# abdur75648/AI-Camera

Hardware: AMD Instinct MI355X
Metric: end-to-end frames/sec @1280x720, 30 persons/frame (higher is better)
Workload: dtype f16

## Files before the change

ai-camera_amd/csrc/conv_plan.cpp:

```cpp
#include "conv_plan.hpp"

#include <algorithm>
#include <cstdlib>

namespace aic {

static int g_conv_cus = 256;
int conv_cu_budget() { return g_conv_cus; }
void set_conv_cu_budget(int cus) { g_conv_cus = std::max(1, cus); }

static long cdiv(long a, long b) { return (a + b - 1) / b; }
static const long B31 = 1l << 31;

static int tile_run(long ntiles, int max_run) {
    int run = 1;
    long best = -1;
    for (int r = 1; r <= max_run; ++r) {
        const long blocks = (ntiles + r - 1) / r, rounds = (blocks + 255) / 256;
        if (r > 1 && rounds < 4) break;
        const long cost = rounds * r;
        if (best < 0 || cost <= best) best = cost, run = r;
    }
    return run;
}
// ... 274 lines not shown

bool conv_x2_supported(int dtype, const ConvArgs& a, int cin2) {
    const int bke = dtype == AIC_F16 ? 32 : 16;
    const int shape = pp_patch_shape(dtype, a);
    if (shape < 2 || a.Cout % 128 || a.w_tail || a.out_f32 || cin2 <= 0 || cin2 % bke) return false;
    return cin2 / bke < a.Cin / bke;
}

int plan_c64_block(const ConvArgs& c1, const ConvArgs& c2, int cu_budget) {
    static const bool on = [] { const char* e = getenv("AICAM_C64_BLOCK"); return !e || atoi(e) != 0; }();
    auto conv64 = [](const ConvArgs& a) {
        return a.KH == 3 && a.KW == 3 && a.stride == 1 && a.pad == 1 && a.Cin == 64 && a.Cout == 64 && !a.out_f32 && a.Kp == 576 && a.act == 2 &&
               a.Ho == a.H && a.Wo == a.W && (a.x_cs | a.x_coff | a.y_cs | a.y_coff) % 8 == 0;
    };
    if (!on || !conv64(c1) || !conv64(c2) || c1.res_mode != 0 || c2.res_mode != 1) return 0;
    if (c1.W != 32 || c1.H % 4 || c1.H != c2.H || c2.W != 32 || c1.M != c2.M || c1.M < 1500000) return 0;
    if (c2.x != c1.y || c2.x_cs != c1.y_cs || c2.x_coff != c1.y_coff) return 0;
    if (c2.res != c1.x || c2.r_cs != c1.x_cs || c2.r_coff != c1.x_coff) return 0;
    if ((long)c1.M * c1.x_cs >= B31 || (long)c2.M * c2.y_cs >= B31) return 0;
    const int n_img = c1.M / (c1.H * c1.W), cus = (cu_budget + 7) / 8 * 8;
    long best = -1;
    int ipb = 0;
    for (int i = 12; i <= 16; ++i) {
        const long blocks = (n_img + i - 1) / i, rounds = (blocks + cus - 1) / cus;
        const long waste = (rounds * cus - blocks) * 1000 / (rounds * cus);
        if (best < 0 || waste < best) best = waste, ipb = i;
    }
    return ipb;
}

bool plan_c2f16(const ConvArgs& c1, const ConvArgs& m1, const ConvArgs& m2, const ConvArgs& c2) {
    static const bool off = getenv("AICAM_NO_C2F") != nullptr;
    if (off) return false;
    auto one = [](const ConvArgs& c, int cin, int cout, int kp) {
        return c.KH == 1 && c.KW == 1 && c.stride == 1 && c.pad == 0 && c.Cin == cin && c.Cout == cout && c.Kp == kp && c.act == 1 &&
               c.res_mode == 0 && !c.out_f32;
    };
    auto three = [](const ConvArgs& c) {
        return c.KH == 3 && c.KW == 3 && c.stride == 1 && c.pad == 1 && c.Cin == 16 && c.Cout == 16 && c.Kp == 160 && c.act == 1 && !c.out_f32;
    };
    if (!one(c1, 32, 32, 32) || !one(c2, 48, 32, 64) || !three(m1) || !three(m2) || m1.res_mode != 0 || m2.res_mode != 2) return false;
    const int H = c1.H, W = c1.W;
    for (const ConvArgs* c : {&c1, &m1, &m2, &c2})
        if (c->H != H || c->W != W || c->Ho != H || c->Wo != W || c->M != c1.M) return false;
    if (H % 8 || W % 32) return false;
    const void* cat = c1.y;
    if (c1.y_coff != 0 || m1.x != cat || m1.x_coff != 16 || m1.x_cs != c1.y_cs || m2.x != m1.y || m2.x_coff != m1.y_coff || m2.x_cs != m1.y_cs ||
        m2.y != cat || m2.y_coff != 32 || m2.res != cat || m2.r_coff != 16 || m2.r_cs != c1.y_cs || c2.x != cat || c2.x_coff != 0 ||
        c2.x_cs != c1.y_cs || c1.y_cs < 48)
        return false;
    return (c1.x_cs | c1.x_coff | c2.y_cs | c2.y_coff) % 8 == 0;
}

}
```

ai-camera_amd/csrc/conv_plan.hpp:

```cpp
#pragma once
#include "assoc_host.hpp"

namespace aic {

struct ConvArgs {
    const void* x;
    const void* w;
    const float* bias;
    void* y;
    const void* res;
    int x_cs, x_coff, H, W, Cin;
    int y_cs, y_coff, Ho, Wo, Cout;
    int r_cs, r_coff, res_mode, act;
    int KH, KW, stride, pad;
    int Kp;
    int M;
    int out_f32;
    int cout_pad;
    unsigned tap_rows;
    const void* zero;
    int xcd_map;
    const float* bias_init;
    const int* n_dev;
    int k_order;
// ... 3 lines not shown
    int xs_cs, xs_coff, Hs, Ws, Cs;
    const void* w_tail;
    const float* b_tail;
    void* y_tail;
    int t_cout, t_kp, t_y_cs, t_y_coff, t_out_f32, t_act;
    float* t_max; int* t_arg;
    int t_hw, t_a0, t_na;
    float* t_box; int t_w, t_stride;
};

int conv_cu_budget();
void set_conv_cu_budget(int cus);

enum class ConvForm {
    Dma,
    Wide,
    Pp,
    PpPatch,
    SpPatch,
    S2Patch,
    Patch,
    PmPatch,
    C16,
    C32s2Tail,
    Stream1x1,
    C64Resident,
};

struct ConvPlan {
    ConvForm form = ConvForm::Dma;
    int mt = 0, nt = 0, wm = 0, wn = 0;
    int nstage = 0;
    int th = 0, tw = 0;
    int cpp = 0, pitch = 0;
    int kord = 0;
    int g = 0;
    bool tail = false;
    bool x2 = false;
    int run = 1;
    long blocks = 0;
};

int conv_k_order(int dtype, const ConvArgs& a);
ConvPlan plan_conv(int dtype, const ConvArgs& a, int cu_budget);

ConvPlan plan_conv_launch(int dtype, ConvArgs& a, int cu_budget);

bool conv_tail_supported(int dtype, const ConvArgs& lead, const ConvArgs& tail);
bool conv_xs_supported(int dtype, const ConvArgs& a, int cs);
bool conv_x2_supported(int dtype, const ConvArgs& a, int cin2);

int plan_c64_block(const ConvArgs& c1, const ConvArgs& c2, int cu_budget);
bool plan_c2f16(const ConvArgs& cv1, const ConvArgs& m_cv1, const ConvArgs& m_cv2, const ConvArgs& cv2);

}
```

ai-camera_amd/csrc/engine.cpp:

```cpp
#include "engine.hpp"

#include <algorithm>
#include <cmath>
#include <cstdlib>
#include <fstream>

namespace aic {

namespace {

struct Reader {
    const char* p;
    size_t n, off = 0;
    template <class T> const T* take(size_t count) {
        AIC_REQUIRE(off + count * sizeof(T) <= n, AIC_ERR_FORMAT, "engine file truncated");
        const T* r = reinterpret_cast<const T*>(p + off);
        off += count * sizeof(T);
        return r;
    }
};

inline int round_up(int v, int m) { return (v + m - 1) / m * m; }

inline uint16_t f32_to_f16_bits(float f) {
// ... 488 lines not shown
    auto conv_args = [&](size_t k) {
        const int* u = ops[k].v;
        const BufDesc& xb = bufs[u[1]];
        const BufDesc& yb = bufs[u[4]];
        const ConvWeights& w = weights[u[15]];
        ConvArgs a{};
        a.x = xb.p, a.w = w.w.p, a.bias = w.bias.p, a.y = yb.p;
        a.x_cs = xb.c, a.x_coff = u[2], a.H = xb.h, a.W = xb.w, a.Cin = w.cin_eff;
        a.y_cs = yb.c, a.y_coff = u[5], a.Ho = yb.h, a.Wo = yb.w, a.Cout = w.cout;
        a.res = nullptr, a.r_cs = 0, a.r_coff = 0, a.res_mode = u[14], a.act = u[11];
        if (u[14]) { a.res = bufs[u[12]].p, a.r_cs = bufs[u[12]].c, a.r_coff = u[13]; }
        a.KH = w.kh, a.KW = w.kw, a.stride = u[9], a.pad = u[10];
        if (ops[k].xs_buf >= 0) {
            const BufDesc& bs = bufs[ops[k].xs_buf];
            a.xs = bs.p, a.xs_cs = bs.c, a.xs_coff = ops[k].xs_coff, a.Hs = bs.h, a.Ws = bs.w, a.Cs = ops[k].xs_c;
        }
        if (u[16]) {
            const BufDesc& b2 = bufs[u[16] - 1];
            a.x2 = b2.p, a.x2_cs = b2.c, a.x2_coff = u[17], a.H2 = b2.h, a.W2 = b2.w, a.s2 = u[19], a.Cin2 = u[18];
            fl += 2.0 * n * yb.h * yb.w * (double)w.cout * u[18];
            by += ((double)n * yb.h * yb.w * u[18] + (double)w.cout * u[18]) * (dtype == AIC_F16 ? 2 : 4);
        }
        a.Kp = w.Kp, a.M = n * yb.h * yb.w, a.out_f32 = yb.f32, a.cout_pad = w.cout_pad, a.zero = d_zero.p;
        a.tap_rows = 0;
        a.n_dev = n_items_dev;
        for (int kh = 0; kh < w.kh; ++kh) a.tap_rows |= 1u << (kh * w.kw);
        AIC_REQUIRE(w.kh * w.kw <= 25, AIC_ERR_FORMAT, "kernel window larger than 5x5");
        fl += 2.0 * a.M * (double)w.cout * w.cin * w.kh * w.kw;
        by += ((double)n * xb.h * xb.w * w.cin + (double)a.M * w.cout) * (dtype == AIC_F16 ? 2 : 4) +
              (double)w.cout * w.cin * w.kh * w.kw * (dtype == AIC_F16 ? 2 : 4);
        return a;
    };
    auto done = [&](int kind, int n_ops) { st.kind = kind, st.n_ops = n_ops, st.fl = fl, st.by = by; return st; };
    const ConvArgs a = st.a[0] = conv_args(oi);
    bool pair = false;
    ConvArgs a2{};
    if (dtype == AIC_F16 && oi + 1 < op1 && ops[oi + 1].v[0] == OP_CONV && ops[oi + 1].fuse == 0 && a.Cin == 64 && a.Cout == 64 &&
        a.res_mode == 0 && ops[oi + 1].v[14] == 1) {
        const double fl0 = fl, by0 = by;
        a2 = conv_args(oi + 1);
        pair = a2.res == a.x && a2.x == a.y;
        if (!pair) fl = fl0, by = by0;
    }
    if (!pair && dtype == AIC_F16 && oi + 3 < op1 && a.KH == 1 && a.Cin == 32 && a.Cout == 32 && ops[oi + 1].v[0] == OP_CONV &&
        ops[oi + 2].v[0] == OP_CONV && ops[oi + 3].v[0] == OP_CONV && !ops[oi + 1].fuse && !ops[oi + 2].fuse && !ops[oi + 3].fuse) {
        const double fl0 = fl, by0 = by;
        const ConvArgs b1 = conv_args(oi + 1), b2 = conv_args(oi + 2), b3 = conv_args(oi + 3);
        if (plan_c2f16(a, b1, b2, b3)) {
            st.a[1] = b1, st.a[2] = b2, st.a[3] = b3;
            return done(ConvStep::C2f16, 4);
        }
        fl = fl0, by = by0;
    }
    if (const int ipb = pair ? plan_c64_block(a, a2, conv_cu_budget()) : 0) {
        st.a[1] = a2, st.ipb = ipb;
        return done(ConvStep::C64Block, 2);
    }
    if (pair) { fl = 0, by = 0; (void)conv_args(oi); }
    if (o.fuse == 3 && oi + 1 < op1) {
        const double fl0 = fl, by0 = by;
        const ConvArgs t = conv_args(oi + 1);
        if (conv_tail_supported(dtype, a, t)) {
            ConvArgs at = a;
            at.w_tail = t.w, at.b_tail = t.bias, at.y_tail = t.y, at.t_cout = t.Cout, at.t_kp = t.Kp;
            at.t_y_cs = t.y_cs, at.t_y_coff = t.y_coff, at.t_out_f32 = t.out_f32, at.t_act = t.act;
            static const bool cls_reduce_on = getenv("AICAM_NO_CLS_REDUCE") == nullptr;
            static const bool box_decode_on = getenv("AICAM_NO_BOX_DECODE") == nullptr;
            if (reduce_cls && kind == KIND_YOLO && t.out_f32 && t.act == 0 && t.y_coff == 0 && t.y_cs == t.Cout) {
                const bool is_cls = cls_reduce_on && t.Cout == meta[0], is_box = box_decode_on && meta[1] == 16 && t.Cout == 64 && a.Cout == 64 && !is_cls;
                int a0 = 0;
                for (size_t l = 0; l < outs.size() && (is_cls || is_box); ++l) {
                    const int* ov = outs[l].v;
                    const BufDesc& ob = bufs[ov[is_cls ? 1 : 0]];
                    if (ob.p == t.y && ov[3] * ov[4] == t.Ho * t.Wo) {
                        at.t_hw = ov[3] * ov[4], at.t_a0 = a0, at.t_na = n_anchors;
                        if (is_cls) {
                            at.t_max = d_maxlogit.p, at.t_arg = d_labels.p;
                            st.cls_bits |= 1u << l;
                        } else {
                            at.t_box = d_boxes.p, at.t_w = ov[4], at.t_stride = ov[2];
                            st.box_bits |= 1u << l;
                        }
                    }
                    a0 += ov[3] * ov[4];
                }
            }
            st.a[0] = at;
            return done(ConvStep::Tail, 2);
        }
        fl = fl0, by = by0;
    }
    return done(ConvStep::Single, 1);
}

void Model::run_range(size_t op0, size_t op1, int n, hipStream_t s) {
    const bool prof_conv = (dev->prof_mask >> PROF_CONV) & 1u;
    bool span_open = false;
    auto span_close = [&] { if (span_open) { dev->prof_end(PROF_CONV, s); span_open = false; } };
    for (size_t oi = op0; oi < op1; ++oi) {
        const OpDesc& o = ops[oi];
        const int* v = o.v;
        const BufDesc& sb = bufs[v[1]];
        const BufDesc& db = bufs[v[4]];
        if (o.fuse == 2) continue;
        if (o.fuse == 1 || v[0] != OP_CONV) span_close();
        if (o.fuse == 1) {
            const ConvWeights& w = weights[v[15]];
            const int* pv = ops[oi + 1].v;
            const BufDesc& pb = bufs[pv[4]];
            const double fl = 2.0 * n * sb.h * sb.w * 64.0 * 27.0;
            Prof pr(*dev, PROF_CONV_DIRECT, s, fl, (double)n * (sb.h * sb.w * 16.0 + pb.h * pb.w * 128.0));
            launch_reid_stem_pool(sb.p, w.w.p, w.bias.p, pb.p, n, sb.h, sb.w, w.Kp, pb.c, pv[5], in_pix4 ? 4 : 8, s,
                                  (crop_src.frames && in_pix4) ? &crop_src : nullptr, n_items_dev);
            continue;
        }
        if (v[0] == OP_CONV) {
            if (prof_conv && !span_open) { dev->prof_begin(PROF_CONV, s, 0, 0); span_open = true; }
            const ConvStep st = conv_step(oi, op1, n);
            if (prof_conv) dev->prof_account(PROF_CONV, st.fl, st.by);
            switch (st.kind) {
                case ConvStep::C2f16: launch_c2f16(st.a[0], st.a[1], st.a[2], st.a[3], s); break;
                case ConvStep::C64Block: launch_c64_block(st.a[0], st.a[1], st.ipb, s); break;
                case ConvStep::Tail: cls_reduced |= st.cls_bits, box_decoded |= st.box_bits; [[fallthrough]];
                default: launch_conv_igemm(dtype, st.a[0], s);
            }
            oi += st.n_ops - 1;
        } else {
            EltArgs a{};
            a.src = sb.p, a.dst = db.p, a.n = n, a.h = sb.h, a.w = sb.w, a.c = v[3];
            if (emb_host_out && oi + 1 == ops.size() && v[0] == OP_L2NORM && v[4] == outs[0].v[0]) a.dst = emb_host_out;
            a.s_cs = sb.c, a.s_coff = v[2], a.d_cs = db.c, a.d_coff = v[5];
            a.n_dev = n_items_dev;
            Prof pr(*dev, PROF_MISC, s, 0, 0);
            switch (v[0]) {
                case OP_SPPF_POOL: launch_sppf_pool(dtype, a, s); break;
                case OP_UPSAMPLE2X: launch_upsample2x(dtype, a, s); break;
                case OP_MAXPOOL3S2: launch_maxpool3s2(dtype, a, s); break;
                case OP_AVGPOOL: launch_avgpool(dtype, a, s); break;
                case OP_L2NORM: launch_l2norm(dtype, a, s); break;
                default: throw Error(AIC_ERR_FORMAT, "unknown op in engine file");
            }
        }
    }
    span_close();
}

DetArgs Model::det_args(int batch, float conf, float iou, int max_det, const LetterboxGeom* g) {
    AIC_REQUIRE(kind == KIND_YOLO, AIC_ERR_INVALID, "not a YOLO engine");
    AIC_REQUIRE(max_det > 0 && max_det <= max_det_cap, AIC_ERR_CAPACITY, "max_det out of range (1..1024)");
    AIC_REQUIRE(conf > 0.f && conf < 1.f, AIC_ERR_INVALID, "conf_thresh must be in (0,1)");
    DetArgs a{};
    int a0 = 0;
    for (size_t l = 0; l < outs.size(); ++l) {
        const int* v = outs[l].v;
        a.lvl[l].box = reinterpret_cast<const float*>(bufs[v[0]].p);
        a.lvl[l].cls = reinterpret_cast<const float*>(bufs[v[1]].p);
        a.lvl[l].stride = v[2], a.lvl[l].h = v[3], a.lvl[l].w = v[4], a.lvl[l].a0 = a0;
        a.lvl[l].cls_reduced = (cls_reduced >> l) & 1u, a.lvl[l].box_decoded = (box_decoded >> l) & 1u;
        a0 += v[3] * v[4];
    }
    a.n_levels = (int)outs.size(), a.n_anchors = n_anchors, a.nc = meta[0], a.reg_max = meta[1], a.batch = batch;
    a.fast_exp = dtype == AIC_F16;
    a.logit_thr = (float)std::log((double)conf / (1.0 - (double)conf));
    a.iou_thr = iou, a.max_det = max_det;
    a.pad_w = g ? g->pad_w : 0.f, a.pad_h = g ? g->pad_h : 0.f, a.ratio = g ? g->ratio : 1.f;
    a.orig_w = g ? g->src_w : in_w, a.orig_h = g ? g->src_h : in_h;
    a.boxes = d_boxes.p, a.max_logit = d_maxlogit.p, a.labels = d_labels.p, a.keys = nullptr;
    a.n_cand = d_ncand.p, a.num_dets = d_numdets.p;
    a.out_boxes = d_out_boxes.p, a.out_boxes_orig = g ? d_out_boxes_orig.p : nullptr;
    a.out_scores = d_out_scores.p, a.out_labels = d_out_labels.p;
    return a;
}

void Model::decode_nms(int batch, float conf, float iou, int max_det, const LetterboxGeom* g, hipStream_t s, char* host_out) {
// ... 412 lines not shown
```

ai-camera_amd/csrc/engine.hpp:

```cpp
#pragma once
#include "kernels.hpp"

#include <algorithm>
#include <memory>
#include <vector>

namespace aic {

enum { OP_CONV = 1, OP_SPPF_POOL = 2, OP_UPSAMPLE2X = 3, OP_MAXPOOL3S2 = 4, OP_AVGPOOL = 5, OP_L2NORM = 6 };
enum { KIND_YOLO = 1, KIND_REID = 2 };

struct BufDesc { int h, w, c, f32; void* p; size_t per_item; int esize; };
struct ConvWeights { DevBuf<char> w; DevBuf<float> bias; int cout, cin, cin_eff, kh, kw, K, Kp, cout_pad; int cin2 = 0; };
struct OpDesc { int v[20]; int fuse = 0; int xs_buf = -1, xs_coff = 0, xs_c = 0; };
struct OutDesc { int v[8]; };

struct Model {
    Device* dev = nullptr;
    int kind = 0, in_h = 0, in_w = 0, dtype = AIC_F16, max_items = 0;
    int meta[8] = {0};
    std::vector<BufDesc> bufs;
    std::vector<DevBuf<char>> storage;
    std::vector<OpDesc> ops;
    std::vector<ConvWeights> weights;
    std::vector<OutDesc> outs;
    double flops_per_item = 0;
    int n_convs = 0, n_anchors = 0, out_dim = 0;

    int max_det_cap = 0;
    DevBuf<float> d_boxes, d_maxlogit, d_out_boxes, d_out_boxes_orig, d_out_scores;
    DevBuf<int> d_labels, d_ncand, d_numdets, d_out_labels;
    DevBuf<float> d_in_f32;
    DevBuf<uint8_t> d_frames;
    DevBuf<float> d_crop_boxes;
    DevBuf<int> d_valid;
    DevBuf<char> d_zero;

    std::shared_ptr<const std::vector<char>> blob_copy;
    Model(Device& d, const void* blob, size_t nbytes, int dtype_, int max_items_);
    void* input() { return bufs[0].p; }
    bool in_pix4 = false;
    CropSrc crop_src{nullptr, 0, 0, nullptr, nullptr, nullptr};
    const int* n_items_dev = nullptr;
    bool reduce_cls = false;
    unsigned cls_reduced = 0, box_decoded = 0;
    bool input_pix4_ok() const;
    int fast_items() const {
        size_t per = 1;
        for (const OpDesc& o : ops) {
            if (o.v[0] != OP_CONV || o.fuse != 0) continue;
            for (int bi : {o.v[1], o.v[4]}) per = std::max(per, bufs[bi].per_item / (size_t)std::max(bufs[bi].esize, 1));
        }
        const size_t n = std::min<size_t>((size_t)max_items, ((1ull << 31) - 1) / per);
        return (int)(n > 64 && n < (size_t)max_items ? n / 64 * 64 : n);
    }
    void run(int n_items, hipStream_t s);
    void run_frames(const uint8_t* frames, int n, const LetterboxGeom& g, hipStream_t s);
    void run_range(size_t op0, size_t op1, int n, hipStream_t s);
    struct ConvStep {
        enum { Single = 0, Tail = 1, C64Block = 2, C2f16 = 3 };
        int kind = Single, n_ops = 1;
        int ipb = 0;
        unsigned cls_bits = 0, box_bits = 0;
        ConvArgs a[4];
        double fl = 0, by = 0;
    };
    ConvStep conv_step(size_t oi, size_t op1, int n) const;
    struct SideHead { size_t a, b, cut; };
    std::vector<SideHead> side_heads;
    hipStream_t side_stream[2] = {nullptr, nullptr};
    hipEvent_t side_fork[2] = {nullptr, nullptr}, side_join[2] = {nullptr, nullptr};
    bool side_ok = false;
    int side_max_items = 2;
    void plan_side_heads();
    void run_ops(size_t op0, int n, hipStream_t s);
    ~Model();
    DetArgs det_args(int batch, float conf, float iou, int max_det, const LetterboxGeom* g);
    void decode_nms(int batch, float conf, float iou, int max_det, const LetterboxGeom* g, hipStream_t s, char* host_out = nullptr);
    PinBuf<char> h_det;
    float* emb_host_out = nullptr;
    PinBuf<char> h_emb;
    const float* embeddings() const { return reinterpret_cast<const float*>(bufs[outs[0].v[0]].p); }
};

}

struct aic_model { aic::Model m; aic_model(aic::Device& d, const void* b, size_t n, int dt, int mi) : m(d, b, n, dt, mi) {} };
```

ai-camera_amd/csrc/kernels.hpp:

```cpp
#pragma once
#include "common.hpp"
#include "conv_plan.hpp"

namespace aic {

typedef _Float16 half_t;

void launch_conv_igemm(int dtype, const ConvArgs& a, hipStream_t s);
void launch_c64_block(const ConvArgs& c1, const ConvArgs& c2, int ipb, hipStream_t s);
void launch_c2f16(const ConvArgs& cv1, const ConvArgs& m_cv1, const ConvArgs& m_cv2, const ConvArgs& cv2, hipStream_t s);

struct LetterboxGeom;
bool launch_yolo_stem_fused(const uint8_t* frames, int n, const LetterboxGeom& g, const void* w, const float* bias, int Kp, void* y,
                            int y_cs, int y_coff, int Ho, int Wo, hipStream_t s);

struct CropSrc { const uint8_t* frames; int fh, fw; const float* boxes; const int* frame_of; int* valid; };
void launch_reid_stem_pool(const void* x, const void* w, const float* bias, void* y, int n, int H, int W, int Kp, int y_cs,
                           int y_coff, int in_stride, hipStream_t s, const CropSrc* crop = nullptr, const int* n_dev = nullptr);
bool reid_stem2_usable(int H, int W);

struct EltArgs {
    const void* src; void* dst;
    int n, h, w, c;
    int s_cs, s_coff, d_cs, d_coff;
    const int* n_dev;
};
void launch_sppf_pool(int dtype, const EltArgs& a, hipStream_t s);
void launch_upsample2x(int dtype, const EltArgs& a, hipStream_t s);
void launch_maxpool3s2(int dtype, const EltArgs& a, hipStream_t s);
void launch_avgpool(int dtype, const EltArgs& a, hipStream_t s);
void launch_l2norm(int dtype, const EltArgs& a, hipStream_t s);
void launch_nchw_to_nhwc8(int dtype, const float* src, void* dst, int n, int h, int w, hipStream_t s);
void launch_copy_f32(const float* src, float* dst, size_t count, hipStream_t s);

struct LetterboxGeom {
    int src_h, src_w, out_h, out_w, unpad_h, unpad_w, top, left;
    float ratio, pad_w, pad_h;
};
LetterboxGeom letterbox_geometry(int h, int w, int out_h, int out_w);
void launch_letterbox(const uint8_t* frames, int n, const LetterboxGeom& g, int mode, int dtype, void* out,
                      hipStream_t s);
void launch_letterbox_u8(const uint8_t* frame, const LetterboxGeom& g, const int color_bgr[3], uint8_t* out, hipStream_t s);
void launch_crop_resize(const uint8_t* frames, int h, int w, const float* boxes, const int* frame_of, int n,
                        const int* n_dev, int out_h, int out_w, int mode, int dtype, void* out, int* valid,
                        hipStream_t s, bool slack = false);

struct HeadLevel { const float* box; const float* cls; int h, w, stride, a0; int cls_reduced, box_decoded; };
struct DetArgs {
    HeadLevel lvl[4];
    int n_levels, n_anchors, nc, reg_max, batch;
    int fast_exp;
    float logit_thr, iou_thr;
    int max_det;
    float pad_w, pad_h, ratio; int orig_w, orig_h;
    float* boxes;
    float* max_logit;
    int* labels;
    unsigned long long* keys;
    int* n_cand;
    int* num_dets;
    float* out_boxes;
    float* out_boxes_orig;
    float* out_scores;
// ... 61 lines not shown
```

ai-camera_amd/csrc/kernels_conv_c2f.hip:

```cpp
#include "conv_common.hpp"

namespace aic {

namespace {

constexpr int TH = 8, TW = 32;
constexpr int XR = TH + 4, XC = TW + 4;
constexpr int TR = TH + 2, TC = TW + 2;
constexpr int PX = XR * XC * 16, PT = (TR * TC * 16 + 255) / 256 * 256, PY = TH * TW * 16;
static_assert(PX % 256 == 0 && PY % 256 == 0, "plane pitch");
__device__ __forceinline__ int x_slot(int p, int g) {
    return (p & ~7) | ((p & 7) ^ (2 * g));
}
static_assert((XR * XC) % 8 == 0, "swizzle group");
constexpr int LDS_X = 0, LDS_T = 0, LDS_Y1 = LDS_T + 2 * PT, LDS_Y0A = 4 * PX, LDS_Y0B = LDS_Y0A + 2 * PY;
constexpr int LDS_BYTES = LDS_Y0B + 2 * PX;
static_assert(LDS_Y1 + 2 * PY <= 4 * PX, "T and Y1 live in X's place");

}

struct C2fArgs {
    const half_t* x; half_t* y;
    const half_t *w1, *w2, *w3, *w4;
    const float *b1, *b2, *b3, *b4;
// ... 110 lines not shown
            const int oyl = 2 * wv + (tile >> 1), oxl = (tile & 1) * 16 + r;
            const int base = LDS_T + (oyl * TC + oxl) * 16;
            floatx4 acc = bi3;
#pragma unroll
            for (int m = 0; m < 5; ++m)
                acc = __builtin_amdgcn_mfma_f32_16x16x32_f16(w3[m], *reinterpret_cast<const half8*>(smem + base + d[m]), acc, 0, 0, 0);
            const half4 res = *reinterpret_cast<const half4*>(smem + LDS_Y0B + (q >> 1) * PX + ((oyl + 2) * XC + oxl + 2) * 16 + (q & 1) * 8);
            half4 o;
#pragma unroll
            for (int e = 0; e < 4; ++e) o[e] = (half_t)(act_fast<1>(acc[e]) + (float)res[e]);
            *reinterpret_cast<half4*>(smem + LDS_Y1 + (q >> 1) * PY + (oyl * TW + oxl) * 16 + (q & 1) * 8) = o;
        }
    }
    __syncthreads();

    half_t* yg = a.y + (size_t)img * a.H * a.W * a.y_cs + a.y_coff;
#pragma unroll
    for (int tile = 0; tile < 4; ++tile) {
        const int oyl = 2 * wv + (tile >> 1), oxl = (tile & 1) * 16 + r;
        const int a0 = q < 2 ? LDS_Y0A + q * PY + (oyl * TW + oxl) * 16 : LDS_Y0B + (q - 2) * PX + ((oyl + 2) * XC + oxl + 2) * 16;
        const half8 x0 = *reinterpret_cast<const half8*>(smem + a0);
        const half8 x1 = *reinterpret_cast<const half8*>(smem + LDS_Y1 + (q & 1) * PY + (oyl * TW + oxl) * 16);
        float v[2][4];
#pragma unroll
        for (int ct = 0; ct < 2; ++ct) {
            floatx4 acc = {0.f, 0.f, 0.f, 0.f};
            acc = __builtin_amdgcn_mfma_f32_16x16x32_f16(w4[ct][0], x0, acc, 0, 0, 0);
            acc = __builtin_amdgcn_mfma_f32_16x16x32_f16(w4[ct][1], x1, acc, 0, 0, 0);
#pragma unroll
            for (int e = 0; e < 4; ++e) v[ct][e] = act_fast<1>(acc[e] + bi4[ct][e]);
        }
        const half8 o = {(half_t)v[0][0], (half_t)v[0][1], (half_t)v[0][2], (half_t)v[0][3],
                         (half_t)v[1][0], (half_t)v[1][1], (half_t)v[1][2], (half_t)v[1][3]};
        *reinterpret_cast<half8*>(yg + ((size_t)(oy0 + oyl) * a.W + ox0 + oxl) * a.y_cs + 8 * q) = o;
    }
}

void launch_c2f16(const ConvArgs& c1, const ConvArgs& m1, const ConvArgs& m2, const ConvArgs& c2, hipStream_t s) {
    static_assert(TH == 8 && TW == 32, "plan_c2f16 checks the map against 8 x 32 tiles");
    const int H = c1.H, W = c1.W;
    C2fArgs a{};
    a.x = reinterpret_cast<const half_t*>(c1.x), a.y = reinterpret_cast<half_t*>(c2.y);
    a.w1 = reinterpret_cast<const half_t*>(c1.w), a.w2 = reinterpret_cast<const half_t*>(m1.w);
    a.w3 = reinterpret_cast<const half_t*>(m2.w), a.w4 = reinterpret_cast<const half_t*>(c2.w);
    a.b1 = c1.bias, a.b2 = m1.bias, a.b3 = m2.bias, a.b4 = c2.bias;
    a.x_cs = c1.x_cs, a.x_coff = c1.x_coff, a.y_cs = c2.y_cs, a.y_coff = c2.y_coff, a.H = H, a.W = W;
    a.n_img = c1.M / (H * W), a.xcd_map = 1;
    set_lds_limit(c2f16_fused_kernel, LDS_BYTES);
    const int tiles_x = W / TW, tiles_y = H / TH;
    hipLaunchKernelGGL(c2f16_fused_kernel, dim3(a.n_img * tiles_x * tiles_y), dim3(256), (size_t)LDS_BYTES, s, a, tiles_x, tiles_y);
    KCHECK();
}

}
```

ai-camera_amd/hip_engine.py:

```python
from __future__ import annotations

import ctypes as C
import os
import time
from pathlib import Path
from typing import Dict, List, NamedTuple, Tuple

import numpy as np

from . import _lib as L
from . import config

TensorInfo = NamedTuple('TensorInfo', [('name', str), ('dtype', object), ('shape', Tuple[int, ...]), ('is_dynamic', bool)])


def _torch():
    import torch
    return torch


class HipEngine:
    default_conf, default_iou, default_max_det = config.YOLO_CONF_THRESHOLD, config.YOLO_NMS_THRESHOLD, config.YOLO_MAX_DET

    def __init__(self, engine_path, device=None, dtype="fp16", max_items=None, warm_up=True):
# ... 54 lines not shown
        try:
            self.close()
        except Exception:
            pass

    def yolo_infer_np(self, images_nchw, conf=None, iou=None, max_det=None):
        x = L.as_f32(images_nchw)
        b = x.shape[0]
        md = int(max_det or self.max_det)
        nd = np.zeros(b, np.int32)
        boxes, scores, labels = np.zeros((b, md, 4), np.float32), np.zeros((b, md), np.float32), np.zeros((b, md), np.int32)
        L.call("aic_yolo_infer", self._h, L.ptr(x), b, L.HOST, float(conf if conf is not None else self.conf_thresh),
               float(iou if iou is not None else self.iou_thresh), md, L.ptr(nd), L.ptr(boxes), L.ptr(scores), L.ptr(labels))
        return nd, boxes, scores, labels

    def yolo_head_np(self, images_nchw):
        x = L.as_f32(images_nchw)
        b = x.shape[0]
        dfl = np.zeros((b, self.n_anchors, 64), np.float32)
        cls = np.zeros((b, self.n_anchors, self.out_dim), np.float32)
        L.call("aic_yolo_head", self._h, L.ptr(x), b, L.HOST, L.ptr(dfl), L.ptr(cls))
        return dfl, cls

    def yolo_decode_np(self, images_nchw):
        x = L.as_f32(images_nchw)
        b = x.shape[0]
        boxes, ml = np.zeros((b, self.n_anchors, 4), np.float32), np.zeros((b, self.n_anchors), np.float32)
        lab = np.zeros((b, self.n_anchors), np.int32)
        L.call("aic_yolo_decode", self._h, L.ptr(x), b, L.HOST, L.ptr(boxes), L.ptr(ml), L.ptr(lab))
        return boxes, ml, lab

    def reid_infer_np(self, crops_nchw):
        x = L.as_f32(crops_nchw)
        n = x.shape[0]
        out = np.zeros((n, self.out_dim), np.float32)
        if n:
            L.call("aic_reid_infer", self._h, L.ptr(x), n, L.HOST, L.ptr(out), L.HOST)
        return out

    def read_buffer_np(self, buf, n):
        with open(self.engine_path, "rb") as f:
            head = np.frombuffer(f.read(68), "<i4")
            tab = np.frombuffer(f.read(16 * int(head[5])), "<i4").reshape(-1, 4)
        h, w, c, f32 = (int(v) for v in tab[buf])
        out = np.empty((int(n), h, w, c), np.float32 if f32 or self.dtype == L.F32 else np.float16)
        L.call("aic_model_read_buffer", self._h, int(buf), L.ptr(out), out.nbytes)
        return out

    def conv_plan(self, op, n):
        out = np.zeros(24, np.int32)
        L.call("aic_model_conv_plan", self._h, int(op), int(n), L.ptr(out))
        names = ["form", "mt", "nt", "wm", "wn", "nstage", "th", "tw", "cpp", "pitch", "kord", "g", "tail", "x2", "run", "blocks"]
        forms = ["Dma", "Wide", "Pp", "PpPatch", "SpPatch", "S2Patch", "Patch", "PmPatch", "C16", "C32s2Tail", "Stream1x1", "C64Resident"]
        r = {"kind": {-2: "covered", -1: "none", 0: "conv", 1: "conv+tail", 2: "c64_block", 3: "c2f16"}[int(out[0])],
             "first_op": int(out[1]), "n_ops": int(out[2]), "ipb": int(out[3])}
        if out[0] in (0, 1):
            r.update({k: int(v) for k, v in zip(names, out[5:21])})
            r.update(form=forms[r["form"]], k_order=int(out[4]), xs=int(out[21]), y_coff=int(out[22]), x_coff=int(out[23]))
        return r

    def detect_np(self, frames_bgr, conf=None, iou=None, max_det=None):
        f = np.ascontiguousarray(frames_bgr, dtype=np.uint8)
        if f.ndim == 3:
            f = f[None]
        b, h, w, _ = f.shape
        md = int(max_det or self.max_det)
        nd = np.zeros(b, np.int32)
        boxes, scores, labels = np.zeros((b, md, 4), np.float32), np.zeros((b, md), np.float32), np.zeros((b, md), np.int32)
        L.call("aic_detect", self._h, L.ptr(f), b, h, w, L.HOST, float(conf if conf is not None else self.conf_thresh),
               float(iou if iou is not None else self.iou_thresh), md, L.ptr(nd), L.ptr(boxes), L.ptr(scores), L.ptr(labels))
        return nd, boxes, scores, labels

    def embed_boxes_np(self, frame_bgr, boxes_xyxy):
        f = np.ascontiguousarray(frame_bgr, dtype=np.uint8)
        b = L.as_f32(boxes_xyxy).reshape(-1, 4)
        n = len(b)
        emb, valid = np.zeros((n, self.out_dim), np.float32), np.zeros(n, np.int32)
        if n:
            L.call("aic_reid_embed", self._h, L.ptr(f), f.shape[0], f.shape[1], L.HOST, L.ptr(b), n, L.ptr(emb), L.ptr(valid))
        return emb, valid

    def _warm_up(self, iterations=5):
        start = time.time()
        n = 1
        x = np.zeros((n, 3, self.in_h, self.in_w), np.float32)
        for _ in range(iterations):
            if self.kind == L.MODEL_YOLO:
                self.yolo_infer_np(x)
            else:
                self.reid_infer_np(x)
        print(f"Warm-up for '{self.engine_path.name}' finished in {time.time() - start:.3f} seconds.")

    def infer(self, inputs: Dict[str, "object"]) -> Dict[str, "object"]:
        torch = _torch()
        info = self.input_info_list[0]
        x = inputs.get(info.name)
        if x is None:
            raise ValueError(f"Missing input: '{info.name}'")
        dev = torch.device(f"cuda:{self.device_index}")
        if x.device != dev:
            x = x.to(dev)
        if x.dtype != torch.float32:
            print(f"Warning: Input tensor '{info.name}' dtype mismatch. Expected {torch.float32}, got {x.dtype}. Casting...")
            x = x.to(torch.float32)
        x = x.contiguous()
        torch.cuda.current_stream(dev).synchronize()
        n = int(x.shape[0])
# ... 31 lines not shown
```

Measured before the change: 12110.

## Fuse 32-channel C2f bottleneck chain and cv2 into one LDS-resident kernel

Adds a fused HIP kernel for C2f blocks with 32-channel bottlenecks (one or two). It chains the 3x3 convs inside LDS using haloed tiles and folds in the final 1x1 cv2, so the intermediate bottleneck tensors never make a round trip to global memory. The engine detects these op chains, checks that the temporary buffers have no other readers, and dispatches the fused kernel by default. In exchange, halo pixels are recomputed for every tile, LDS use is large (which may limit occupancy), and the intermediate concat slices are no longer written out.

Measured after the change: 12080. Within noise of the previous version (-0.3%).

```diff
diff --git a/ai-camera_amd/csrc/conv_plan.cpp b/ai-camera_amd/csrc/conv_plan.cpp
--- a/ai-camera_amd/csrc/conv_plan.cpp
+++ b/ai-camera_amd/csrc/conv_plan.cpp
@@ -350,4 +350,51 @@
     return (c1.x_cs | c1.x_coff | c2.y_cs | c2.y_coff) % 8 == 0;
 }
 
-}
+C2f32Tile c2f32_tile(int nb) {
+    return nb == 2 ? C2f32Tile{8, 16, 4} : C2f32Tile{16, 16, 4};
+}
+
+int plan_c2f32(int dtype, const ConvArgs* cv, int n_convs) {
+    static const int forms = [] {
+        if (getenv("AICAM_NO_C2F32")) return 0;
+        const char* e = getenv("AICAM_C2F32");
+        return e ? atoi(e) : 1;
+    }();
+    if (dtype != AIC_F16 || !cv || (n_convs != 3 && n_convs != 5)) return 0;
+    const int nb = (n_convs - 1) / 2;
+    if (!((forms >> (nb - 1)) & 1)) return 0;
+    const ConvArgs& c2 = cv[n_convs - 1];
+    const int H = c2.H, W = c2.W, M = c2.M;
+    auto plain = [&](const ConvArgs& c) {
+        return c.act == 1 && !c.out_f32 && c.stride == 1 && c.H == H && c.W == W && c.Ho == H && c.Wo == W && c.M == M && !c.xs && !c.x2 &&
+               !c.w_tail && !c.n_dev && !c.bias_init && c.x && c.y && c.w && c.bias;
+    };
+    auto three = [&](const ConvArgs& c) {
+        return plain(c) && c.KH == 3 && c.KW == 3 && c.pad == 1 && c.Cin == 32 && c.Cout == 32 && c.Kp == 288 && c.cout_pad >= 32 &&
+               conv_k_order(AIC_F16, c) == 0;
+    };
+    if (!plain(c2) || c2.KH != 1 || c2.KW != 1 || c2.pad != 0 || c2.Cin != 32 * (nb + 2) || c2.Kp != c2.Cin || c2.Cout != 64 ||
+        c2.cout_pad < 64 || c2.res_mode != 0 || conv_k_order(AIC_F16, c2) != 0)
+        return 0;
+    if (H <= 0 || W <= 0 || M <= 0 || M % (H * W)) return 0;
+    const void* cat = c2.x;
+    const int cs = c2.x_cs;
+    if (c2.x_coff != 0 || cs < 32 * (nb + 2)) return 0;
+    const bool shortcut = cv[1].res_mode == 2;
+    for (int b = 0; b < nb; ++b) {
+        const ConvArgs &m1 = cv[2 * b], &m2 = cv[2 * b + 1];
+        if (!three(m1) || !three(m2) || m1.res_mode != 0 || m2.res_mode != (shortcut ? 2 : 0)) return 0;
+        if (m1.x != cat || m1.x_cs != cs || m1.x_coff != 32 * (b + 1)) return 0;
+        if (m1.y == cat || m2.x != m1.y || m2.x_cs != m1.y_cs || m2.x_coff != m1.y_coff) return 0;
+        if (m2.y != cat || m2.y_cs != cs || m2.y_coff != 32 * (b + 2)) return 0;
+        if (shortcut && (m2.res != cat || m2.r_cs != cs || m2.r_coff != 32 * (b + 1))) return 0;
+    }
+    if (c2.y == cat) return 0;
+    const C2f32Tile t = c2f32_tile(nb);
+    if (H % t.th || W % t.tw) return 0;
+    if ((cs | c2.y_cs | c2.y_coff) % 8) return 0;
+    if ((long)M * cs >= B31 || (long)M * c2.y_cs >= B31) return 0;
+    return nb;
+}
+
+}
diff --git a/ai-camera_amd/csrc/conv_plan.hpp b/ai-camera_amd/csrc/conv_plan.hpp
--- a/ai-camera_amd/csrc/conv_plan.hpp
+++ b/ai-camera_amd/csrc/conv_plan.hpp
@@ -79,5 +79,8 @@
 
 int plan_c64_block(const ConvArgs& c1, const ConvArgs& c2, int cu_budget);
 bool plan_c2f16(const ConvArgs& cv1, const ConvArgs& m_cv1, const ConvArgs& m_cv2, const ConvArgs& cv2);
+int plan_c2f32(int dtype, const ConvArgs* convs, int n_convs);
+struct C2f32Tile { int th, tw, nw; };
+C2f32Tile c2f32_tile(int nb);
 
 }
diff --git a/ai-camera_amd/csrc/engine.cpp b/ai-camera_amd/csrc/engine.cpp
--- a/ai-camera_amd/csrc/engine.cpp
+++ b/ai-camera_amd/csrc/engine.cpp
@@ -564,6 +564,28 @@
         }
         fl = fl0, by = by0;
     }
+    if (!pair && dtype == AIC_F16 && a.KH == 3 && a.Cin == 32 && a.Cout == 32 && a.res_mode == 0 && o.fuse == 0) {
+        for (int nb = 2; nb >= 1; --nb) {
+            const size_t nc = 2 * (size_t)nb + 1;
+            if (oi + nc > op1) continue;
+            bool chain = true;
+            for (size_t k = oi + 1; k < oi + nc; ++k) chain = chain && ops[k].v[0] == OP_CONV && ops[k].fuse == 0;
+            if (!chain) continue;
+            const int tmp = ops[oi].v[4], cat = ops[oi].v[1];
+            for (size_t k = 0; k < ops.size() && chain; ++k) {
+                if ((k >= oi && k < oi + nc) || ops[k].fuse == 2) continue;
+                const int* u = ops[k].v;
+                for (int bi : {tmp, cat})
+                    if (u[1] == bi || (u[0] == OP_CONV && ((u[14] && u[12] == bi) || (u[16] && u[16] - 1 == bi))) || ops[k].xs_buf == bi) chain = false;
+            }
+            for (const auto& ov : outs) chain = chain && ov.v[0] != tmp && ov.v[0] != cat && (kind != KIND_YOLO || (ov.v[1] != tmp && ov.v[1] != cat));
+            if (!chain) continue;
+            const double fl0 = fl, by0 = by;
+            for (size_t k = 1; k < nc; ++k) st.a[k] = conv_args(oi + k);
+            if (plan_c2f32(dtype, st.a, (int)nc) == nb) return done(ConvStep::C2f32, (int)nc);
+            fl = fl0, by = by0;
+        }
+    }
     if (const int ipb = pair ? plan_c64_block(a, a2, conv_cu_budget()) : 0) {
         st.a[1] = a2, st.ipb = ipb;
         return done(ConvStep::C64Block, 2);
@@ -632,6 +654,7 @@
             if (prof_conv) dev->prof_account(PROF_CONV, st.fl, st.by);
             switch (st.kind) {
                 case ConvStep::C2f16: launch_c2f16(st.a[0], st.a[1], st.a[2], st.a[3], s); break;
+                case ConvStep::C2f32: launch_c2f32(st.a, (st.n_ops - 1) / 2, s); break;
                 case ConvStep::C64Block: launch_c64_block(st.a[0], st.a[1], st.ipb, s); break;
                 case ConvStep::Tail: cls_reduced |= st.cls_bits, box_decoded |= st.box_bits; [[fallthrough]];
                 default: launch_conv_igemm(dtype, st.a[0], s);
diff --git a/ai-camera_amd/csrc/engine.hpp b/ai-camera_amd/csrc/engine.hpp
--- a/ai-camera_amd/csrc/engine.hpp
+++ b/ai-camera_amd/csrc/engine.hpp
@@ -58,11 +58,11 @@
     void run_frames(const uint8_t* frames, int n, const LetterboxGeom& g, hipStream_t s);
     void run_range(size_t op0, size_t op1, int n, hipStream_t s);
     struct ConvStep {
-        enum { Single = 0, Tail = 1, C64Block = 2, C2f16 = 3 };
+        enum { Single = 0, Tail = 1, C64Block = 2, C2f16 = 3, C2f32 = 4 };
         int kind = Single, n_ops = 1;
         int ipb = 0;
         unsigned cls_bits = 0, box_bits = 0;
-        ConvArgs a[4];
+        ConvArgs a[5];
         double fl = 0, by = 0;
     };
     ConvStep conv_step(size_t oi, size_t op1, int n) const;
diff --git a/ai-camera_amd/csrc/kernels.hpp b/ai-camera_amd/csrc/kernels.hpp
--- a/ai-camera_amd/csrc/kernels.hpp
+++ b/ai-camera_amd/csrc/kernels.hpp
@@ -9,6 +9,7 @@
 void launch_conv_igemm(int dtype, const ConvArgs& a, hipStream_t s);
 void launch_c64_block(const ConvArgs& c1, const ConvArgs& c2, int ipb, hipStream_t s);
 void launch_c2f16(const ConvArgs& cv1, const ConvArgs& m_cv1, const ConvArgs& m_cv2, const ConvArgs& cv2, hipStream_t s);
+void launch_c2f32(const ConvArgs* convs, int nb, hipStream_t s);
 
 struct LetterboxGeom;
 bool launch_yolo_stem_fused(const uint8_t* frames, int n, const LetterboxGeom& g, const void* w, const float* bias, int Kp, void* y,
diff --git a/ai-camera_amd/csrc/kernels_conv_c2f.hip b/ai-camera_amd/csrc/kernels_conv_c2f.hip
--- a/ai-camera_amd/csrc/kernels_conv_c2f.hip
+++ b/ai-camera_amd/csrc/kernels_conv_c2f.hip
@@ -186,4 +186,226 @@
     KCHECK();
 }
 
-}
+namespace {
+
+constexpr int c2f32_npix(int th, int tw, int h) { return (th + 2 * h) * (tw + 2 * h); }
+constexpr int c2f32_pitch(int th, int tw, int h) { return (c2f32_npix(th, tw, h) * 16 + 255) / 256 * 256; }
+constexpr int c2f32_lds(int nb, int th, int tw) {
+    return 4 * (c2f32_pitch(th, tw, 2 * nb) + c2f32_pitch(th, tw, 2 * nb - 1) + (nb == 2 ? c2f32_pitch(th, tw, 2) : 0));
+}
+
+struct C2f32Args {
+    const half_t* cat;
+    half_t* y;
+    const half_t* w3[4];
+    const float* b3[4];
+    const half_t* wc;
+    const float* bc;
+    int cs, y_cs, y_coff, H, W, shortcut, xcd_map;
+};
+
+struct C2f32W { half8 f[2][9]; floatx4 b[2]; };
+
+__device__ __forceinline__ void c2f32_weights(C2f32W& w, const half_t* wg, const float* bias, int r, int q) {
+#pragma unroll
+    for (int j = 0; j < 2; ++j) {
+        const half_t* wr = wg + (size_t)perm_row<2>(j, r) * 288 + 8 * q;
+#pragma unroll
+        for (int tap = 0; tap < 9; ++tap) w.f[j][tap] = *reinterpret_cast<const half8*>(wr + 32 * tap);
+    }
+    w.b[0] = *reinterpret_cast<const floatx4*>(bias + 8 * q);
+    w.b[1] = *reinterpret_cast<const floatx4*>(bias + 8 * q + 4);
+}
+
+__device__ __forceinline__ half8 c2f32_out(const floatx4 (&acc)[2], const floatx4 (&b)[2], bool sc, const half8& res) {
+    float v[8];
+#pragma unroll
+    for (int e = 0; e < 8; ++e) v[e] = act_fast<1>(acc[e >> 2][e & 3] + b[e >> 2][e & 3]);
+    if (sc) {
+#pragma unroll
+        for (int e = 0; e < 8; ++e) v[e] = v[e] + (float)res[e];
+    }
+    return half8{(half_t)v[0], (half_t)v[1], (half_t)v[2], (half_t)v[3], (half_t)v[4], (half_t)v[5], (half_t)v[6], (half_t)v[7]};
+}
+
+template <int TH, int TW, int NW, int HIN, int HRES>
+__device__ __forceinline__ void c2f32_conv(char* smem, int in, int out, int res, bool sc, const half_t* wg, const float* bias, int oy0, int ox0,
+                                           int H, int W, int wv, int r, int q) {
+    constexpr int HOUT = HIN - 1, WIN = TW + 2 * HIN, WOUT = TW + 2 * HOUT, NP = c2f32_npix(TH, TW, HOUT), NT = (NP + 15) / 16;
+    constexpr int PIN = c2f32_pitch(TH, TW, HIN), POUT = c2f32_pitch(TH, TW, HOUT), PRES = c2f32_pitch(TH, TW, HRES);
+    constexpr int WRES = TW + 2 * HRES, DR = HRES - HOUT;
+    C2f32W w;
+    c2f32_weights(w, wg, bias, r, q);
+    for (int tp = wv; 2 * tp < NT; tp += NW) {
+        int p[2], pr[2], pc[2];
+        half8 xf[2][9];
+#pragma unroll
+        for (int i = 0; i < 2; ++i) {
+            p[i] = min((2 * tp + i) * 16 + r, NP - 1);
+            pr[i] = p[i] / WOUT, pc[i] = p[i] - pr[i] * WOUT;
+            const char* base = smem + in + q * PIN + (pr[i] * WIN + pc[i]) * 16;
+#pragma unroll
+            for (int tap = 0; tap < 9; ++tap) xf[i][tap] = *reinterpret_cast<const half8*>(base + ((tap / 3) * WIN + tap % 3) * 16);
+        }
+        floatx4 acc[2][2];
+#pragma unroll
+        for (int i = 0; i < 2; ++i)
+#pragma unroll
+            for (int j = 0; j < 2; ++j) acc[i][j] = floatx4{0.f, 0.f, 0.f, 0.f};
+#pragma unroll
+        for (int tap = 0; tap < 9; ++tap)
+#pragma unroll
+            for (int i = 0; i < 2; ++i)
+#pragma unroll
+                for (int j = 0; j < 2; ++j) acc[i][j] = __builtin_amdgcn_mfma_f32_16x16x32_f16(w.f[j][tap], xf[i][tap], acc[i][j], 0, 0, 0);
+#pragma unroll
+        for (int i = 0; i < 2; ++i) {
+            const bool inside = (unsigned)(oy0 - HOUT + pr[i]) < (unsigned)H && (unsigned)(ox0 - HOUT + pc[i]) < (unsigned)W;
+            half8 rh = {};
+            if (sc) rh = *reinterpret_cast<const half8*>(smem + res + q * PRES + ((pr[i] + DR) * WRES + pc[i] + DR) * 16);
+            half8 o = c2f32_out(acc[i], w.b, sc, rh);
+            if (!inside) o = half8{};
+            if ((2 * tp + i) * 16 + r < NP) *reinterpret_cast<half8*>(smem + out + q * POUT + p[i] * 16) = o;
+        }
+    }
+}
+
+}
+
+template <int NB, int TH, int TW, int NW>
+__global__ __launch_bounds__(64 * NW) void c2f32_fused_kernel(const C2f32Args a, int tiles_x, int tiles_y) {
+    static_assert((NB == 1 || NB == 2) && (TH * TW) % 16 == 0, "whole 16-pixel tiles of the block's own pixels");
+    constexpr int H0 = 2 * NB, NTHR = 64 * NW;
+    constexpr int PA = c2f32_pitch(TH, TW, H0), PB = c2f32_pitch(TH, TW, H0 - 1);
+    constexpr int LA = 0, LB = 4 * PA, LC = LB + 4 * PB;
+    extern __shared__ __attribute__((aligned(16))) char smem[];
+    const int t = threadIdx.x, lane = t & 63, wv = __builtin_amdgcn_readfirstlane(t >> 6), r = lane & 15, q = lane >> 4;
+    int bx = xcd_tile((int)blockIdx.x, (int)gridDim.x, a.xcd_map);
+    const int tx = bx % tiles_x; bx /= tiles_x;
+    const int ty = bx % tiles_y;
+    const int img = bx / tiles_y;
+    const int oy0 = ty * TH, ox0 = tx * TW;
+    const half_t* cg = a.cat + (size_t)img * a.H * a.W * a.cs;
+
+    {
+        constexpr int WA = TW + 2 * H0, NSLOT = c2f32_npix(TH, TW, H0) * 4, NIT = (NSLOT + NTHR - 1) / NTHR;
+        uint4 v[NIT];
+        int dst[NIT];
+#pragma unroll
+        for (int u = 0; u < NIT; ++u) {
+            const int idx = t + u * NTHR;
+            const int g = idx & 3, p = idx >> 2;
+            const int pr = p / WA, pc = p - pr * WA;
+            const int iy = oy0 - H0 + pr, ix = ox0 - H0 + pc;
+            v[u] = make_uint4(0u, 0u, 0u, 0u);
+            if (idx < NSLOT && (unsigned)iy < (unsigned)a.H && (unsigned)ix < (unsigned)a.W)
+                v[u] = *reinterpret_cast<const uint4*>(cg + ((size_t)iy * a.W + ix) * a.cs + 32 + g * 8);
+            dst[u] = idx < NSLOT ? LA + g * PA + p * 16 : -1;
+        }
+#pragma unroll
+        for (int u = 0; u < NIT; ++u)
+            if (dst[u] >= 0) *reinterpret_cast<uint4*>(smem + dst[u]) = v[u];
+    }
+    __syncthreads();
+    const bool sc = a.shortcut != 0;
+    int l_t, l_prev;
+    if constexpr (NB == 2) {
+        c2f32_conv<TH, TW, NW, 4, 4>(smem, LA, LB, 0, false, a.w3[0], a.b3[0], oy0, ox0, a.H, a.W, wv, r, q);
+        __syncthreads();
+        c2f32_conv<TH, TW, NW, 3, 4>(smem, LB, LC, LA, sc, a.w3[1], a.b3[1], oy0, ox0, a.H, a.W, wv, r, q);
+        __syncthreads();
+        c2f32_conv<TH, TW, NW, 2, 2>(smem, LC, LA, 0, false, a.w3[2], a.b3[2], oy0, ox0, a.H, a.W, wv, r, q);
+        l_t = LA, l_prev = LC;
+    } else {
+        c2f32_conv<TH, TW, NW, 2, 2>(smem, LA, LB, 0, false, a.w3[0], a.b3[0], oy0, ox0, a.H, a.W, wv, r, q);
+        l_t = LB, l_prev = LA;
+    }
+    __syncthreads();
+
+    {
+        constexpr int KS = NB + 2, WT = TW + 2, WP = TW + 4, PT = c2f32_pitch(TH, TW, 1), PP = c2f32_pitch(TH, TW, 2), NT = TH * TW / 16;
+        C2f32W w;
+        c2f32_weights(w, a.w3[2 * NB - 1], a.b3[2 * NB - 1], r, q);
+        half8 wc[4][KS];
+#pragma unroll
+        for (int j = 0; j < 4; ++j)
+#pragma unroll
+            for (int s = 0; s < KS; ++s) wc[j][s] = *reinterpret_cast<const half8*>(a.wc + (size_t)perm_row<4>(j, r) * (32 * KS) + 32 * s + 8 * q);
+        floatx4 bc[4];
+#pragma unroll
+        for (int pp = 0; pp < 2; ++pp) {
+            bc[2 * pp] = *reinterpret_cast<const floatx4*>(a.bc + 32 * pp + 8 * q);
+            bc[2 * pp + 1] = *reinterpret_cast<const floatx4*>(a.bc + 32 * pp + 8 * q + 4);
+        }
+        half_t* yg = a.y + (size_t)img * a.H * a.W * a.y_cs + a.y_coff;
+        for (int tile = wv; tile < NT; tile += NW) {
+            const int p = tile * 16 + r;
+            const int oyl = p / TW, oxl = p - oyl * TW;
+            const int gp = (oy0 + oyl) * a.W + ox0 + oxl;
+            half8 xk[KS];
+            xk[0] = *reinterpret_cast<const half8*>(cg + (size_t)gp * a.cs + 8 * q);
+            xk[1] = *reinterpret_cast<const half8*>(cg + (size_t)gp * a.cs + 32 + 8 * q);
+            const int own2 = q * PP + ((oyl + 2) * WP + oxl + 2) * 16;
+            if constexpr (NB == 2) xk[2] = *reinterpret_cast<const half8*>(smem + l_prev + own2);
+            const char* base = smem + l_t + q * PT + (oyl * WT + oxl) * 16;
+            half8 xf[9];
+#pragma unroll
+            for (int tap = 0; tap < 9; ++tap) xf[tap] = *reinterpret_cast<const half8*>(base + ((tap / 3) * WT + tap % 3) * 16);
+            floatx4 acc[2] = {floatx4{0.f, 0.f, 0.f, 0.f}, floatx4{0.f, 0.f, 0.f, 0.f}};
+#pragma unroll
+            for (int tap = 0; tap < 9; ++tap)
+#pragma unroll
+                for (int j = 0; j < 2; ++j) acc[j] = __builtin_amdgcn_mfma_f32_16x16x32_f16(w.f[j][tap], xf[tap], acc[j], 0, 0, 0);
+            half8 rh = {};
+            if (sc) rh = *reinterpret_cast<const half8*>(smem + l_prev + own2);
+            xk[KS - 1] = c2f32_out(acc, w.b, sc, rh);
+            floatx4 acc2[4];
+#pragma unroll
+            for (int j = 0; j < 4; ++j) acc2[j] = floatx4{0.f, 0.f, 0.f, 0.f};
+#pragma unroll
+            for (int s = 0; s < KS; ++s)
+#pragma unroll
+                for (int j = 0; j < 4; ++j) acc2[j] = __builtin_amdgcn_mfma_f32_16x16x32_f16(wc[j][s], xk[s], acc2[j], 0, 0, 0);
+            half8 o[2];
+#pragma unroll
+            for (int pp = 0; pp < 2; ++pp) {
+                float v[8];
+#pragma unroll
+                for (int e = 0; e < 8; ++e) v[e] = act_fast<1>(acc2[2 * pp + (e >> 2)][e & 3] + bc[2 * pp + (e >> 2)][e & 3]);
+                o[pp] = half8{(half_t)v[0], (half_t)v[1], (half_t)v[2], (half_t)v[3], (half_t)v[4], (half_t)v[5], (half_t)v[6], (half_t)v[7]};
+            }
+#pragma unroll
+            for (int pp = 0; pp < 2; ++pp) *reinterpret_cast<half8*>(yg + (size_t)gp * a.y_cs + 32 * pp + 8 * q) = o[pp];
+        }
+    }
+}
+
+template <int NB, int TH, int TW, int NW>
+static void launch_c2f32_t(const C2f32Args& a, int n_img, hipStream_t s) {
+    constexpr int lds = c2f32_lds(NB, TH, TW);
+    static_assert(lds <= 160 * 1024, "LDS of one CU");
+    set_lds_limit(c2f32_fused_kernel<NB, TH, TW, NW>, lds);
+    const int tiles_x = a.W / TW, tiles_y = a.H / TH;
+    hipLaunchKernelGGL((c2f32_fused_kernel<NB, TH, TW, NW>), dim3((unsigned)(n_img * tiles_x * tiles_y)), dim3(64 * NW), (size_t)lds, s, a, tiles_x, tiles_y);
+    KCHECK();
+}
+
+void launch_c2f32(const ConvArgs* cv, int nb, hipStream_t s) {
+    AIC_REQUIRE(nb == 1 || nb == 2, AIC_ERR_INVALID, "c2f32: one or two bottlenecks");
+    const ConvArgs& c2 = cv[2 * nb];
+    C2f32Args a{};
+    a.cat = reinterpret_cast<const half_t*>(c2.x), a.y = reinterpret_cast<half_t*>(c2.y);
+    for (int i = 0; i < 2 * nb; ++i) a.w3[i] = reinterpret_cast<const half_t*>(cv[i].w), a.b3[i] = cv[i].bias;
+    a.wc = reinterpret_cast<const half_t*>(c2.w), a.bc = c2.bias;
+    a.cs = c2.x_cs, a.y_cs = c2.y_cs, a.y_coff = c2.y_coff, a.H = c2.H, a.W = c2.W, a.shortcut = cv[1].res_mode == 2, a.xcd_map = 1;
+    const int n_img = c2.M / (c2.H * c2.W);
+    const C2f32Tile t = c2f32_tile(nb);
+    const int key = nb * 1000000 + t.th * 10000 + t.tw * 100 + t.nw;
+    switch (key) {
+        case 2081604: launch_c2f32_t<2, 8, 16, 4>(a, n_img, s); break;
+        case 1161604: launch_c2f32_t<1, 16, 16, 4>(a, n_img, s); break;
+        default: AIC_REQUIRE(false, AIC_ERR_INVALID, "c2f32: no instantiation for this tile");
+    }
+}
+
+}
diff --git a/ai-camera_amd/hip_engine.py b/ai-camera_amd/hip_engine.py
--- a/ai-camera_amd/hip_engine.py
+++ b/ai-camera_amd/hip_engine.py
@@ -130,7 +130,7 @@
         L.call("aic_model_conv_plan", self._h, int(op), int(n), L.ptr(out))
         names = ["form", "mt", "nt", "wm", "wn", "nstage", "th", "tw", "cpp", "pitch", "kord", "g", "tail", "x2", "run", "blocks"]
         forms = ["Dma", "Wide", "Pp", "PpPatch", "SpPatch", "S2Patch", "Patch", "PmPatch", "C16", "C32s2Tail", "Stream1x1", "C64Resident"]
-        r = {"kind": {-2: "covered", -1: "none", 0: "conv", 1: "conv+tail", 2: "c64_block", 3: "c2f16"}[int(out[0])],
+        r = {"kind": {-2: "covered", -1: "none", 0: "conv", 1: "conv+tail", 2: "c64_block", 3: "c2f16", 4: "c2f32"}[int(out[0])],
              "first_op": int(out[1]), "n_ops": int(out[2]), "ipb": int(out[3])}
         if out[0] in (0, 1):
             r.update({k: int(v) for k, v in zip(names, out[5:21])})
```
